# Bergvca/string_grouper

Hardware: NVIDIA H100
Metric: match_strings matched pairs/sec (663k names self-match @0.8, top 20, 3-gram) (higher is better)
Workload: dtype f64

## Files before the change

### string_grouper_b200/csrc/sg_cossim.cu

```cuda
#include <cub/cub.cuh>
#include <cuda_fp16.h>

#include "sg_common.cuh"

namespace sg {

constexpr int PB_THREADS = 1024;
constexpr int PB_ITEMS = 8;
constexpr int PB_CAP = PB_THREADS * PB_ITEMS;
constexpr size_t PB_SMEM = (size_t)PB_CAP * 8;

__device__ __forceinline__ uint32_t make_posting(float v, float w_scale, uint32_t local) {
    return ((uint32_t)__half_as_ushort(__float2half_rn(v * w_scale)) << 16) | local;
}

__global__ void postings_tile_count_kernel(int64_t n_rows, int64_t T, int W, const int64_t *__restrict__ indptr,
                                           const int32_t *__restrict__ perm, int32_t *__restrict__ tile_cnt) {
    const int64_t t = (int64_t)blockIdx.x * (blockDim.x >> 5) + (threadIdx.x >> 5);
    if (t > T) return;
    int s = 0;
    if (t < T) {
        const int64_t p1 = (t + 1) * W < n_rows ? (t + 1) * W : n_rows;
        for (int64_t p = t * W + lane_id(); p < p1; p += 32) {
            const int64_t row = perm ? perm[p] : p;
            s += (int)(indptr[row + 1] - indptr[row]);
        }
    }
#pragma unroll
    for (int o = 16; o; o >>= 1) s += __shfl_xor_sync(FULL, s, o);
    if (lane_id() == 0) tile_cnt[t] = s;
}

__device__ __forceinline__ void postings_emit_runs(const uint32_t *keys, const uint32_t *pst, int n, int start,
                                                   int64_t t, int64_t T, int64_t Tp, int2 *__restrict__ dir,
                                                   unsigned short *__restrict__ maxw_rows) {
    for (int i = threadIdx.x; i < n; i += blockDim.x) {
        const uint32_t f = keys[i];
        if (i > 0 && keys[i - 1] == f) continue;
        uint32_t m = 0;
        int j = i;
        for (; j < n && keys[j] == f; ++j) m = max(m, (pst[j] >> 16) & 0x7fffu);
        dir[(int64_t)f * T + t] = make_int2(start + i, (int)(((uint32_t)(j - i) & 0xffffu) | (m << 16)));
        maxw_rows[(int64_t)f * Tp + t] = (unsigned short)m;
    }
}

template <int ITEMS>
__device__ __forceinline__ void postings_sort_tile(uint32_t *skey, uint32_t *spost, int n, int key_bits) {
    typedef cub::BlockRadixSort<uint32_t, PB_THREADS, ITEMS, uint32_t> Sort;
    static_assert(sizeof(typename Sort::TempStorage) <= PB_SMEM, "block sort scratch exceeds the tile buffers");
    const uint32_t pad = (uint32_t)((1ull << key_bits) - 1);
    uint32_t keys[ITEMS], vals[ITEMS];
#pragma unroll
    for (int k = 0; k < ITEMS; ++k) {
        const int i = k * PB_THREADS + threadIdx.x;
        keys[k] = i < n ? skey[i] : pad;
        vals[k] = i < n ? spost[i] : 0u;
    }
    __syncthreads();
    Sort(*reinterpret_cast<typename Sort::TempStorage *>(skey)).SortBlockedToStriped(keys, vals, 0, key_bits);
    __syncthreads();
#pragma unroll
    for (int k = 0; k < ITEMS; ++k) {
        const int i = k * PB_THREADS + threadIdx.x;
        skey[i] = keys[k];
        spost[i] = vals[k];
    }
}

__global__ void __launch_bounds__(PB_THREADS)
postings_tile_build_kernel(int64_t n_rows, int64_t T, int64_t Tp, int W, int key_bits,
                           const int64_t *__restrict__ indptr, const int32_t *__restrict__ indices,
                           const float *__restrict__ val, const int32_t *__restrict__ perm, float w_scale,
                           const int32_t *__restrict__ tile_off, uint32_t *__restrict__ post, int2 *__restrict__ dir,
                           unsigned short *__restrict__ maxw_rows, uint32_t *__restrict__ big_key,
                           uint32_t *__restrict__ big_post, int32_t *__restrict__ big_end, int32_t *n_spilled) {
    typedef cub::BlockScan<int, PB_THREADS> Scan;
    __shared__ typename Scan::TempStorage scan_tmp;
    __shared__ int64_t row_p0[PB_THREADS];
    __shared__ int row_off[PB_THREADS];
    extern __shared__ __align__(16) uint32_t pb_smem[];
    uint32_t *skey = pb_smem, *spost = pb_smem + PB_CAP;

    const int64_t t = blockIdx.x;
    const int off0 = tile_off[t], n = tile_off[t + 1] - off0;
    const bool big = n > PB_CAP;
    if (threadIdx.x == 0) {
        big_end[t] = big ? off0 + n : off0;
        if (big && n_spilled) atomicAdd(n_spilled, 1);
    }
    uint32_t *kdst = big ? big_key + off0 : skey, *pdst = big ? big_post + off0 : spost;

    const int64_t p0 = t * W;
    const int nr = (int)((p0 + W < n_rows ? p0 + W : n_rows) - p0);
    int base = 0;
    for (int r0 = 0; r0 < nr; r0 += PB_THREADS) {
        const int r = r0 + threadIdx.x;
        int len = 0;
        int64_t q = 0;
        if (r < nr) {
            const int64_t row = perm ? perm[p0 + r] : p0 + r;
            q = indptr[row];
            len = (int)(indptr[row + 1] - q);
        }
        int o, total;
        Scan(scan_tmp).ExclusiveSum(len, o, total);
        row_p0[threadIdx.x] = q;
        row_off[threadIdx.x] = o;
        __syncthreads();
#pragma unroll 4
        for (int j = threadIdx.x; j < total; j += PB_THREADS) {
            int k = 0;
#pragma unroll
            for (int s = PB_THREADS / 2; s; s >>= 1)
                if (row_off[k + s] <= j) k += s;
            const int64_t p = row_p0[k] + (j - row_off[k]);
            kdst[base + j] = (uint32_t)indices[p];
            pdst[base + j] = make_posting(val[p], w_scale, (uint32_t)(r0 + k));
        }
        base += total;
        __syncthreads();
    }
    if (big) return;

    if (n <= PB_THREADS * 2) postings_sort_tile<2>(skey, spost, n, key_bits);
    else if (n <= PB_THREADS * 4) postings_sort_tile<4>(skey, spost, n, key_bits);
    else postings_sort_tile<PB_ITEMS>(skey, spost, n, key_bits);
    __syncthreads();
    for (int i = threadIdx.x; i < n; i += PB_THREADS) post[off0 + i] = spost[i];
    postings_emit_runs(skey, spost, n, off0, t, T, Tp, dir, maxw_rows);
}

__global__ void __launch_bounds__(256)
postings_big_dir_kernel(int64_t T, int64_t Tp, const int32_t *__restrict__ tile_off,
                        const int32_t *__restrict__ big_end, const uint32_t *keys, const uint32_t *pst, uint32_t *post,
                        int2 *__restrict__ dir, unsigned short *__restrict__ maxw_rows) {
    const int64_t t = blockIdx.x;
    const int off0 = tile_off[t], n = big_end[t] - off0;
    if (n == 0) return;
    if (pst != post)
        for (int i = threadIdx.x; i < n; i += blockDim.x) post[off0 + i] = pst[off0 + i];
    postings_emit_runs(keys + off0, pst + off0, n, off0, t, T, Tp, dir, maxw_rows);
}

__device__ __forceinline__ float post_w(uint32_t e) { return __half2float(__ushort_as_half((unsigned short)(e >> 16))); }
__device__ __forceinline__ int post_c(uint32_t e) { return (int)(e & 0xffffu); }

__device__ __forceinline__ int dir_len(int2 d) { return d.y & 0xffff; }
__device__ __forceinline__ float dir_maxw(int2 d) {
    return __half2float(__ushort_as_half((unsigned short)((unsigned)d.y >> 16)));
}

constexpr int LONG_BUCKET = 64;
#ifndef SG_WALK_MLP
#define SG_WALK_MLP 1
#endif
#ifndef SG_FILTER_MLP
#define SG_FILTER_MLP 1
#endif

constexpr int min_ctas(int nw) { return nw == 32 ? 2 : nw == 16 ? 3 : nw == 8 ? 5 : 8; }

constexpr float FIX_ONE = 32768.f;

template <typename AccT>
struct AccOps;
template <>
struct AccOps<float> {
    typedef float val_t;
    static constexpr int PER16 = 4;
    static __device__ __forceinline__ float left_weight(float a) { return a; }
    static __device__ __forceinline__ float threshold(float thr) { return thr; }
    static __device__ __forceinline__ float fma_store(float *acc, int col, float a, float w) {
        const float v = fmaf(a, w, acc[col]);
        acc[col] = v;
        return v;
    }
    static __device__ __forceinline__ float atomic_add(float *acc, int col, float a, float w) {
        const float x = a * w;
        return atomicAdd(acc + col, x) + x;
    }
    static __device__ __forceinline__ float vmax(float a, float b) { return fmaxf(a, b); }
    static __device__ __forceinline__ unsigned above(const uint4 &v, float thr) {
        return (__uint_as_float(v.x) > thr ? 1u : 0u) | (__uint_as_float(v.y) > thr ? 2u : 0u) |
               (__uint_as_float(v.z) > thr ? 4u : 0u) | (__uint_as_float(v.w) > thr ? 8u : 0u);
    }
    static __device__ __forceinline__ float value(const uint4 &v, int i) {
        return __uint_as_float(i < 2 ? (i == 0 ? v.x : v.y) : (i == 2 ? v.z : v.w));
    }
};
template <>
struct AccOps<uint16_t> {
    typedef int val_t;
    static constexpr int PER16 = 8;
    static __device__ __forceinline__ float left_weight(float a) { return a * FIX_ONE; }
    static __device__ __forceinline__ int threshold(float thr) { return (int)floorf(thr * FIX_ONE); }
    static __device__ __forceinline__ int atomic_add(uint16_t *acc, int col, float a, float w) {
        const int x = __float2int_rn(a * w);
        const unsigned sh = ((unsigned)col & 1u) << 4;
        const unsigned old = atomicAdd(reinterpret_cast<unsigned *>(acc) + (col >> 1), (unsigned)x << sh);
        return (int)((old >> sh) & 0xffffu) + x;
    }
    static __device__ __forceinline__ int fma_store(uint16_t *acc, int col, float a, float w) {
        return atomic_add(acc, col, a, w);
    }
    static __device__ __forceinline__ int vmax(int a, int b) { return max(a, b); }
    static __device__ __forceinline__ unsigned pair_above(unsigned u, int thr) {
        return ((int)(u & 0xffffu) > thr ? 1u : 0u) | ((int)(u >> 16) > thr ? 2u : 0u);
    }
    static __device__ __forceinline__ unsigned above(const uint4 &v, int thr) {
        return pair_above(v.x, thr) | (pair_above(v.y, thr) << 2) | (pair_above(v.z, thr) << 4) |
               (pair_above(v.w, thr) << 6);
    }
    static __device__ __forceinline__ float value(const uint4 &v, int i) {
        const unsigned w = i < 4 ? (i < 2 ? v.x : v.y) : (i < 6 ? v.z : v.w);
        return (float)((w >> ((i & 1) << 4)) & 0xffffu) * (1.f / FIX_ONE);
    }
};

template <typename AccT>
__device__ __forceinline__ void apply_buckets(AccT *__restrict__ acc, const uint32_t *__restrict__ post, int b0,
                                              int len, float a, int lane,
                                              typename AccOps<AccT>::val_t &seen) {
    typedef AccOps<AccT> Ops;
    unsigned m = __ballot_sync(FULL, len >= LONG_BUCKET);
    while (m) {
        const int src = __ffs(m) - 1;
        m &= m - 1;
        const int s = __shfl_sync(FULL, b0, src);
        const int e = s + __shfl_sync(FULL, len, src);
        const float ak = __shfl_sync(FULL, a, src);
        int p = s + lane;
        for (; p + 96 < e; p += 128) {
            const uint32_t e0 = post[p], e1 = post[p + 32], e2 = post[p + 64], e3 = post[p + 96];
            const typename Ops::val_t v0 = Ops::fma_store(acc, post_c(e0), ak, post_w(e0));
            const typename Ops::val_t v1 = Ops::fma_store(acc, post_c(e1), ak, post_w(e1));
            const typename Ops::val_t v2 = Ops::fma_store(acc, post_c(e2), ak, post_w(e2));
            const typename Ops::val_t v3 = Ops::fma_store(acc, post_c(e3), ak, post_w(e3));
            seen = Ops::vmax(Ops::vmax(Ops::vmax(seen, v0), Ops::vmax(v1, v2)), v3);
        }
        for (; p < e; p += 32) {
            const uint32_t e0 = post[p];
            seen = Ops::vmax(seen, Ops::fma_store(acc, post_c(e0), ak, post_w(e0)));
        }
        __syncwarp();
    }
    const int ln = len >= LONG_BUCKET ? 0 : len;
    int incl = ln;
#pragma unroll
    for (int o = 1; o < 32; o <<= 1) {
        const int up = __shfl_up_sync(FULL, incl, o);
        if (lane >= o) incl += up;
    }
    const int total = __shfl_sync(FULL, incl, 31);
    const int d = b0 - (incl - ln);
    for (int base = 0; base < total; base += 32 * SG_WALK_MLP) {
        uint32_t e[SG_WALK_MLP];
        float ak[SG_WALK_MLP];
#pragma unroll
        for (int u = 0; u < SG_WALK_MLP; ++u) {
            const int item = base + 32 * u + lane;
            int k = 0;
#pragma unroll
            for (int st = 16; st; st >>= 1) {
                const int v = __shfl_sync(FULL, incl, k + st - 1);
                if (v <= item) k += st;
            }
            const int dk = __shfl_sync(FULL, d, k);
            ak[u] = __shfl_sync(FULL, a, k);
            e[u] = 0u;
            if (item < total) e[u] = post[dk + item];
        }
#pragma unroll
        for (int u = 0; u < SG_WALK_MLP; ++u) {
            const int item = base + 32 * u + lane;
            if (item < total) seen = Ops::vmax(seen, Ops::atomic_add(acc, post_c(e[u]), ak[u], post_w(e[u])));
        }
    }
    __syncwarp();
}

struct FloorArgs {
    float *floor;
    const int32_t *self_rank;
    int seed, top_n;
    float margin, margin_pf;
};

__device__ __forceinline__ void floor_merge(float &kept, float x, int lane) {
#pragma unroll
    for (int k = 2; k <= 32; k <<= 1) {
#pragma unroll
        for (int j = k >> 1; j > 0; j >>= 1) {
            const float o = __shfl_xor_sync(FULL, x, j);
            x = (((lane & k) == 0) == ((lane & j) == 0)) ? fminf(x, o) : fmaxf(x, o);
        }
    }
    kept = fmaxf(kept, x);
#pragma unroll
    for (int j = 16; j > 0; j >>= 1) {
        const float o = __shfl_xor_sync(FULL, kept, j);
        kept = (lane & j) == 0 ? fmaxf(kept, o) : fminf(kept, o);
    }
}

template <int NW, typename AccT, bool FLOOR, bool RANGE = false>
__device__ __forceinline__ void
candidates_body(const int64_t *__restrict__ a_indptr, const int32_t *__restrict__ a_len,
                const int32_t *__restrict__ a_idx, const float *__restrict__ a_val, int64_t row_begin,
                int64_t row_end, const int32_t *__restrict__ perm_a, int64_t n_right,
                const int2 *__restrict__ bdir, const uint32_t *__restrict__ maxw_h,
                const uint32_t *__restrict__ post, const int32_t *__restrict__ perm_b, int Tp, int W,
                int64_t T, int64_t tiles_per_group, float a_scale, float thr_all,
                const float *__restrict__ thr_row, const float *__restrict__ xp_norm,
                const float *__restrict__ tile_bound, const int32_t *__restrict__ diag_rank,
                const unsigned long long *__restrict__ group_items, int32_t *__restrict__ cand_row,
                int32_t *__restrict__ cand_col, float *__restrict__ cand_partial, unsigned long long cap,
                unsigned long long *__restrict__ cand_count, unsigned long long *__restrict__ row_queue,
                const FloorArgs &fa, const int32_t *__restrict__ hi_pos = nullptr) {
    typedef AccOps<AccT> Ops;
    typedef typename Ops::val_t val_t;
    extern __shared__ __align__(16) unsigned char smem_raw[];
    const int lane = threadIdx.x & 31;
    const int warp = threadIdx.x >> 5;
    AccT *acc = reinterpret_cast<AccT *>(smem_raw) + (size_t)warp * W;
    uint4 *acc16 = reinterpret_cast<uint4 *>(acc);
    const int n16 = W / Ops::PER16;
    const uint4 zero4 = make_uint4(0u, 0u, 0u, 0u);

    for (int c = lane; c < n16; c += 32) acc16[c] = zero4;
    __syncwarp();

    const int64_t n_rows = row_end - row_begin;
    const int64_t n_groups = (T + tiles_per_group - 1) / tiles_per_group;
    unsigned long long n_items =
        group_items ? group_items[n_groups] : (unsigned long long)n_rows * (unsigned long long)n_groups;
    if constexpr (FLOOR) {
        if (fa.self_rank) n_items = (unsigned long long)n_rows * (unsigned long long)(fa.seed ? 1 : n_groups - 1);
    }
    const int n_tiles = (int)T;
    int64_t group = 0;
    for (;;) {
        unsigned long long item = 0;
        if (lane == 0) item = atomicAdd(row_queue, 1ull);
        item = __shfl_sync(FULL, item, 0);
        if (item >= n_items) break;
        int64_t ridx;
        if (group_items) {
            while (item >= group_items[group + 1]) ++group;
            ridx = (int64_t)(item - group_items[group]);
            if constexpr (RANGE) ridx += (int64_t)group_items[n_groups + 1 + group];
        } else {
            group = (int64_t)(item / (unsigned long long)n_rows);
            ridx = (int64_t)(item % (unsigned long long)n_rows);
        }
        const int64_t row = perm_a ? perm_a[ridx] : row_begin + ridx;
        int own_batch = 0;
        if constexpr (FLOOR) {
            if (fa.self_rank) {
                const int64_t pos = fa.self_rank[row];
                const int64_t own = pos / (tiles_per_group * W);
                if (fa.seed) {
                    group = own;
                    own_batch = (int)((pos / W - own * tiles_per_group) >> 6);
                } else if (group >= own) {
                    ++group;
                }
            }
        }
        const int64_t p0 = a_indptr[row];
        const int nf = a_len ? a_len[row] : (int)(a_indptr[row + 1] - p0);
        if (nf == 0) continue;
        float thr_r = thr_row ? thr_row[row] : thr_all;
        float e_r = 0.f, kept = 0.f, floor_seen = 0.f;
        if constexpr (FLOOR) e_r = __fmaf_ru(fa.margin_pf, (float)nf, fa.margin);
        const float xp = xp_norm ? xp_norm[row] : 0.f;
        const int t_begin = (int)(group * tiles_per_group);
        int t_end = (int)(t_begin + tiles_per_group < T ? t_begin + tiles_per_group : T);
        const int dr = diag_rank ? diag_rank[row] : 0;
        int hr = 0;
        if constexpr (RANGE) {
            hr = hi_pos[row];
            const int t_hi = (int)(((int64_t)hr + W - 1) / W);
            if (t_hi < t_end) t_end = t_hi;
        }
        const int t_first = (int)(((int64_t)dr / W) & ~63);
        const int tb_begin = t_first > t_begin ? t_first : t_begin;

        int f0 = 0;
        float a0 = 0.f;
        __half2 a2 = __float2half2_rn(0.f);
        if (lane < nf) {
            f0 = a_idx[p0 + lane];
            const float a = a_val[p0 + lane] * a_scale;
            a0 = Ops::left_weight(a);
            a2 = __half2half2(__float2half_ru(fabsf(a)));
        }
        const int2 *drow = bdir + f0 * n_tiles;
        const int nk = nf < 32 ? nf : 32;
        const float slack = 5e-4f * (float)nf + 1e-4f;

        for (int tb0 = tb_begin; tb0 < t_end; tb0 += 64) {
            int tb = tb0;
            if constexpr (FLOOR) {
                tb += own_batch * 64;
                if (tb >= t_end) tb -= (t_end - tb_begin + 63) / 64 * 64;
                const float f = __shfl_sync(FULL, __ldcg(fa.floor + row), 0);
                if (f > floor_seen) {
                    floor_seen = f;
                    thr_r = fmaxf(thr_r, __fsub_rd(__fsub_rd(f, e_r), FLOOR_EPS));
                }
            }
            unsigned m_even, m_odd;
            const int t0 = tb + 2 * lane;
            const bool up0 = (t0 + 1) * W > dr, up1 = (t0 + 2) * W > dr;
            {
                __half2 ub2 = __float2half2_rn(0.f);
                const uint32_t *mrow = maxw_h + (tb >> 1) + lane;
                for (int k0 = 0; k0 < nk; k0 += SG_FILTER_MLP) {
                    uint32_t m[SG_FILTER_MLP];
                    __half2 ak2[SG_FILTER_MLP];
#pragma unroll
                    for (int u = 0; u < SG_FILTER_MLP; ++u) {
                        const int kk = k0 + u;
                        const int fk = __shfl_sync(FULL, f0, kk & 31);
                        ak2[u] = __shfl_sync(FULL, a2, kk & 31);
                        m[u] = kk < nk ? mrow[fk * (Tp >> 1)] : 0u;
                    }
#pragma unroll
                    for (int u = 0; u < SG_FILTER_MLP; ++u)
                        ub2 = __hfma2(ak2[u], *reinterpret_cast<const __half2 *>(&m[u]), ub2);
                }
                for (int base = 32; base < nf; base += 32) {
                    int fl = 0;
                    __half2 al = __float2half2_rn(0.f);
                    if (base + lane < nf) {
                        fl = a_idx[p0 + base + lane];
                        al = __half2half2(__float2half_ru(fabsf(a_val[p0 + base + lane] * a_scale)));
                    }
                    const int nc = nf - base < 32 ? nf - base : 32;
                    for (int kk = 0; kk < nc; ++kk) {
                        const int fk = __shfl_sync(FULL, fl, kk);
                        const __half2 ak = __shfl_sync(FULL, al, kk);
                        const uint32_t mv = mrow[fk * (Tp >> 1)];
                        ub2 = __hfma2(ak, *reinterpret_cast<const __half2 *>(&mv), ub2);
                    }
                }
                const float2 ub = __half22float2(ub2);
                const float2 tb2 = reinterpret_cast<const float2 *>(tile_bound)[(tb >> 1) + lane];
                const float thr0 = xp > 0.f ? fmaxf(fmaf(-xp, tb2.x, thr_r), 0.f) : thr_r;
                const float thr1 = xp > 0.f ? fmaxf(fmaf(-xp, tb2.y, thr_r), 0.f) : thr_r;
                m_even = __ballot_sync(FULL, t0 < t_end && up0 && ub.x + slack > thr0);
                m_odd = __ballot_sync(FULL, t0 + 1 < t_end && up1 && ub.y + slack > thr1);
            }
            int t = -1;
            if (m_even) { t = tb + 2 * (__ffs(m_even) - 1); m_even &= m_even - 1; }
            else if (m_odd) { t = tb + 2 * (__ffs(m_odd) - 1) + 1; m_odd &= m_odd - 1; }
            int2 d_cur = make_int2(0, 0);
            if (t >= 0 && lane < nf) d_cur = drow[t];
            while (t >= 0) {
                int t_next = -1;
                if (m_even) { t_next = tb + 2 * (__ffs(m_even) - 1); m_even &= m_even - 1; }
                else if (m_odd) { t_next = tb + 2 * (__ffs(m_odd) - 1) + 1; m_odd &= m_odd - 1; }
                int2 d_next = make_int2(0, 0);
                if (t_next >= 0 && lane < nf) d_next = drow[t_next];

                const float thr_f = xp > 0.f ? fmaxf(fmaf(-xp, tile_bound[t], thr_r), 0.f) : thr_r;
                const val_t thr_c = Ops::threshold(thr_f);
                val_t seen = 0;
                apply_buckets<AccT>(acc, post, d_cur.x, dir_len(d_cur), a0, lane, seen);
                if (nf > 32) {
                    for (int base = 32; base < nf; base += 32) {
                        const int k = base + lane;
                        int b0 = 0, len = 0;
                        float a = 0.f;
                        if (k < nf) {
                            const int2 d = bdir[a_idx[p0 + k] * n_tiles + t];
                            a = Ops::left_weight(a_val[p0 + k] * a_scale);
                            b0 = d.x;
                            len = dir_len(d);
                        }
                        apply_buckets<AccT>(acc, post, b0, len, a, lane, seen);
                    }
                }
                if (!__any_sync(FULL, seen > thr_c)) {
                    for (int c = lane; c < n16; c += 32) acc16[c] = zero4;
                } else {
                    for (int c0 = 0; c0 < n16; c0 += 32) {
                        const int c = c0 + lane;
                        unsigned m = 0;
                        uint4 v = zero4;
                        if (c < n16) {
                            v = acc16[c];
                            if (v.x | v.y | v.z | v.w) {
                                acc16[c] = zero4;
                                m = Ops::above(v, thr_c);
                                const int below = dr - (t * W + c * Ops::PER16);
                                if (below > 0) m = below >= Ops::PER16 ? 0u : m & (~0u << below);
                                if constexpr (RANGE) {
                                    const int room = hr - (t * W + c * Ops::PER16);
                                    if (room < Ops::PER16) m = room <= 0 ? 0u : m & ((1u << room) - 1u);
                                }
                            }
                        }
                        if constexpr (FLOOR) {
                            float best = 0.f;
                            for (unsigned mm = m; mm; mm &= mm - 1) best = fmaxf(best, Ops::value(v, __ffs(mm) - 1));
                            const float lb = fmaxf(__fsub_rd(best, e_r), 0.f);
                            if (__any_sync(FULL, lb > __shfl_sync(FULL, kept, fa.top_n - 1))) {
                                floor_merge(kept, lb, lane);
                                const float kth = __shfl_sync(FULL, kept, fa.top_n - 1);
                                if (kth > floor_seen) {
                                    floor_seen = kth;
                                    if (lane == 0) atomicMax(reinterpret_cast<int *>(fa.floor + row), __float_as_int(kth));
                                    thr_r = fmaxf(thr_r, __fsub_rd(__fsub_rd(kth, e_r), FLOOR_EPS));
                                }
                            }
                        }
                        if (__any_sync(FULL, m != 0)) {
                            const int cnt = __popc(m);
                            int incl = cnt;
#pragma unroll
                            for (int o = 1; o < 32; o <<= 1) {
                                const int up = __shfl_up_sync(FULL, incl, o);
                                if (lane >= o) incl += up;
                            }
                            unsigned long long slot = 0;
                            if (lane == 31) slot = atomicAdd(cand_count, (unsigned long long)incl);
                            slot = __shfl_sync(FULL, slot, 31) + (unsigned long long)(incl - cnt);
                            while (m) {
                                const int i = __ffs(m) - 1;
                                m &= m - 1;
                                if (slot < cap) {
                                    const int col = t * W + c * Ops::PER16 + i;
                                    cand_row[slot] = (int32_t)row;
                                    cand_col[slot] = perm_b ? perm_b[col] : col;
                                    if (cand_partial) cand_partial[slot] = Ops::value(v, i);
                                }
                                ++slot;
                            }
                        }
                    }
                }
                __syncwarp();
                t = t_next;
                d_cur = d_next;
            }
        }
    }
}

#define SG_CAND_PARAMS                                                                                              \
    const int64_t *__restrict__ a_indptr, const int32_t *__restrict__ a_len, const int32_t *__restrict__ a_idx,     \
        const float *__restrict__ a_val, int64_t row_begin, int64_t row_end, const int32_t *__restrict__ perm_a,    \
        int64_t n_right, const int2 *__restrict__ bdir, const uint32_t *__restrict__ maxw_h,                        \
        const uint32_t *__restrict__ post, const int32_t *__restrict__ perm_b, int Tp, int W, int64_t T,            \
        int64_t tiles_per_group, float a_scale, float thr_all, const float *__restrict__ thr_row,                   \
        const float *__restrict__ xp_norm, const float *__restrict__ tile_bound,                                    \
        const int32_t *__restrict__ diag_rank, const unsigned long long *__restrict__ group_items,                  \
        int32_t *__restrict__ cand_row, int32_t *__restrict__ cand_col, float *__restrict__ cand_partial,           \
        unsigned long long cap, unsigned long long *__restrict__ cand_count,                                        \
        unsigned long long *__restrict__ row_queue
#define SG_CAND_ARGS                                                                                              \
    a_indptr, a_len, a_idx, a_val, row_begin, row_end, perm_a, n_right, bdir, maxw_h, post, perm_b, Tp, W, T,     \
        tiles_per_group, a_scale, thr_all, thr_row, xp_norm, tile_bound, diag_rank, group_items, cand_row,        \
        cand_col, cand_partial, cap, cand_count, row_queue

template <int NW, typename AccT>
__global__ void __launch_bounds__(NW * 32, min_ctas(NW)) cossim_candidates_kernel(SG_CAND_PARAMS) {
    candidates_body<NW, AccT, false>(SG_CAND_ARGS, FloorArgs{});
}

template <int NW, typename AccT>
__global__ void __launch_bounds__(NW * 32, min_ctas(NW)) cossim_candidates_floor_kernel(SG_CAND_PARAMS, FloorArgs fa) {
    candidates_body<NW, AccT, true>(SG_CAND_ARGS, fa);
}

template <int NW, typename AccT>
__global__ void __launch_bounds__(NW * 32, min_ctas(NW))
    cossim_candidates_range_kernel(SG_CAND_PARAMS, const int32_t *__restrict__ hi_pos) {
    candidates_body<NW, AccT, false, true>(SG_CAND_ARGS, FloorArgs{}, hi_pos);
}
#undef SG_CAND_PARAMS
#undef SG_CAND_ARGS

__global__ void diag_last_kernel(int64_t n_rows, const int32_t *__restrict__ perm_a, int64_t row_begin,
                                 const int32_t *__restrict__ diag_rank, int64_t group_cols,
                                 unsigned long long *__restrict__ last) {
    const int64_t ridx = (int64_t)blockIdx.x * blockDim.x + threadIdx.x;
    long long g = -1;
    if (ridx < n_rows) g = diag_rank[perm_a ? perm_a[ridx] : row_begin + ridx] / group_cols;
    const unsigned peers = __match_any_sync(FULL, g);
    if (g >= 0 && lane_id() == 31 - __clz(peers)) atomicMax(last + g, (unsigned long long)(ridx + 1));
}

__global__ void diag_items_kernel(int64_t n_groups, unsigned long long *__restrict__ items) {
    const int lane = threadIdx.x;
    unsigned long long run_max = 0, run_sum = 0;
    for (int64_t g0 = 0; g0 < n_groups; g0 += 32) {
        const int64_t g = g0 + lane;
        unsigned long long v = g < n_groups ? items[g] : 0ull;
#pragma unroll
        for (int o = 1; o < 32; o <<= 1) {
            const unsigned long long up = __shfl_up_sync(FULL, v, o);
            if (lane >= o && up > v) v = up;
        }
        if (run_max > v) v = run_max;
        run_max = __shfl_sync(FULL, v, 31);
        if (g >= n_groups) v = 0;
        unsigned long long s = v;
#pragma unroll
        for (int o = 1; o < 32; o <<= 1) {
            const unsigned long long up = __shfl_up_sync(FULL, s, o);
            if (lane >= o) s += up;
        }
        if (g < n_groups) items[g] = run_sum + s - v;
        run_sum += __shfl_sync(FULL, s, 31);
    }
    if (lane == 0) items[n_groups] = run_sum;
}

__global__ void range_groups_kernel(int64_t n_rows, const int32_t *__restrict__ perm_a, int64_t row_begin,
                                    const int32_t *__restrict__ lo_pos, const int32_t *__restrict__ hi_pos,
                                    int64_t group_cols, int64_t n_groups, unsigned long long *__restrict__ items) {
    const int64_t ridx = (int64_t)blockIdx.x * blockDim.x + threadIdx.x;
    long long g0 = -1, g1 = -1;
    if (ridx < n_rows) {
        const int64_t row = perm_a ? perm_a[ridx] : row_begin + ridx;
        const int64_t lo = lo_pos[row], hi = hi_pos[row];
        if (hi > lo) {
            g0 = lo / group_cols;
            g1 = (hi - 1) / group_cols;
        }
    }
    unsigned peers = __match_any_sync(FULL, g0);
    if (g0 >= 0 && lane_id() == 31 - __clz(peers)) atomicMax(items + g0, (unsigned long long)(ridx + 1));
    peers = __match_any_sync(FULL, g1);
    if (g1 >= 0 && lane_id() == __ffs(peers) - 1)
        atomicMax(items + n_groups + 1 + g1, (unsigned long long)(n_rows - ridx));
}

__global__ void range_items_kernel(int64_t n_rows, int64_t n_groups, unsigned long long *__restrict__ items) {
    const int lane = threadIdx.x;
    unsigned long long *first = items + n_groups + 1;
    unsigned long long run = 0;
    for (int64_t g0 = 0; g0 < n_groups; g0 += 32) {
        const int64_t g = n_groups - 1 - g0 - lane;
        unsigned long long v = g >= 0 ? first[g] : 0ull;
#pragma unroll
        for (int o = 1; o < 32; o <<= 1) {
            const unsigned long long up = __shfl_up_sync(FULL, v, o);
            if (lane >= o && up > v) v = up;
        }
        if (run > v) v = run;
        run = __shfl_sync(FULL, v, 31);
        if (g >= 0) first[g] = (unsigned long long)n_rows - v;
    }
    unsigned long long run_max = 0, run_sum = 0;
    for (int64_t g0 = 0; g0 < n_groups; g0 += 32) {
        const int64_t g = g0 + lane;
        unsigned long long v = g < n_groups ? items[g] : 0ull;
#pragma unroll
        for (int o = 1; o < 32; o <<= 1) {
            const unsigned long long up = __shfl_up_sync(FULL, v, o);
            if (lane >= o && up > v) v = up;
        }
        if (run_max > v) v = run_max;
        run_max = __shfl_sync(FULL, v, 31);
        const unsigned long long c = (g < n_groups && v > first[g]) ? v - first[g] : 0ull;
        unsigned long long s = c;
#pragma unroll
        for (int o = 1; o < 32; o <<= 1) {
            const unsigned long long up = __shfl_up_sync(FULL, s, o);
            if (lane >= o) s += up;
        }
        if (g < n_groups) items[g] = run_sum + s - c;
        run_sum += __shfl_sync(FULL, s, 31);
    }
    if (lane == 0) items[n_groups] = run_sum;
}

template <typename T>
struct ExactOps;
template <>
struct ExactOps<double> {
    static __device__ __forceinline__ double mul(double a, double b) { return __dmul_rn(a, b); }
    static __device__ __forceinline__ double add(double a, double b) { return __dadd_rn(a, b); }
};
template <>
struct ExactOps<float> {
    static __device__ __forceinline__ float mul(float a, float b) { return __fmul_rn(a, b); }
    static __device__ __forceinline__ float add(float a, float b) { return __fadd_rn(a, b); }
};

template <typename T>
__device__ __forceinline__ T merge_dot(const int32_t *__restrict__ ai, const T *__restrict__ av, int64_t pa,
                                       int64_t ea, const int32_t *__restrict__ bi,
                                       const T *__restrict__ bv, int64_t pb, int64_t eb) {
    T sum = (T)0;
    if (pa >= ea || pb >= eb) return sum;
    int32_t fa = ai[pa], fb = bi[pb];
    for (;;) {
        if (fa == fb) {
            sum = ExactOps<T>::add(sum, ExactOps<T>::mul(av[pa], bv[pb]));
            ++pa;
            ++pb;
            if (pa >= ea || pb >= eb) break;
            fa = ai[pa];
            fb = bi[pb];
        } else if (fa < fb) {
            if (++pa >= ea) break;
            fa = ai[pa];
        } else {
            if (++pb >= eb) break;
            fb = bi[pb];
        }
    }
    return sum;
}

template <typename T>
__device__ __forceinline__ T merge_dot_vec(const int32_t *__restrict__ ai, const T *__restrict__ av, int64_t pa,
                                           int64_t ea, const int32_t *__restrict__ bi,
                                           const T *__restrict__ bv, int64_t pb, int64_t eb) {
    T sum = (T)0;
    if (pa >= ea || pb >= eb) return sum;
    const int32_t END = 0x7fffffff;
    int32_t fa = ai[pa];
    for (int64_t k = pb & ~(int64_t)3; k < eb; k += 4) {
        int32_t f[4];
        if (k + 4 <= eb) {
            const int4 q = __ldg(reinterpret_cast<const int4 *>(bi + k));
            f[0] = q.x, f[1] = q.y, f[2] = q.z, f[3] = q.w;
        } else {
#pragma unroll
            for (int j = 0; j < 4; ++j) f[j] = k + j < eb ? bi[k + j] : END;
        }
#pragma unroll
        for (int j = 0; j < 4; ++j) {
            const int64_t p = k + j;
            if (p < pb || p >= eb) continue;
            const int32_t fb = f[j];
            while (fa < fb) {
                if (++pa >= ea) return sum;
                fa = ai[pa];
            }
            if (fa == fb) sum = ExactOps<T>::add(sum, ExactOps<T>::mul(av[pa], bv[p]));
        }
    }
    return sum;
}

__device__ __forceinline__ void keep_pairs(bool keep, bool mir, int32_t r, int32_t c, double sc, int lane,
                                           int32_t *__restrict__ keep_row, int32_t *__restrict__ keep_col,
                                           double *__restrict__ out, unsigned long long *__restrict__ keep_count,
                                           unsigned long long *__restrict__ mirror_count,
                                           int32_t *__restrict__ row_cnt, int64_t row_begin) {
    const unsigned m = __ballot_sync(FULL, keep);
    if (!m) return;
    const unsigned mm = __ballot_sync(FULL, mir);
    const int leader = __ffs(m) - 1;
    unsigned long long base = 0;
    if (lane == leader) {
        base = atomicAdd(keep_count, (unsigned long long)(__popc(m) + __popc(mm)));
        if (mm) atomicAdd(mirror_count, (unsigned long long)__popc(mm));
    }
// ... 891 lines not shown
```

Measured before the change: 218.1 million.

## Widen block-max filter to four tiles per lane in non-floor path

Generalizes the tile upper-bound filter so each lane evaluates TPL tiles (4 when FLOOR is off, 2 when on), loading maxw entries as uint2 and doing two half2 FMAs per feature. This halves the number of filter iterations and shuffles per tile when FLOOR is off, and widens the per-lane loads. It also adds an SG_BLOCKMAX_ONLY compile-time probe that counts passing tiles. The risks are more registers and a changed order of candidate tiles. The FLOOR path still steps own_batch by 64 while BATCH is 64 there, so that path is unchanged in size.

```diff
diff --git a/string_grouper_b200/csrc/sg_cossim.cu b/string_grouper_b200/csrc/sg_cossim.cu
--- a/string_grouper_b200/csrc/sg_cossim.cu
+++ b/string_grouper_b200/csrc/sg_cossim.cu
@@ -1,5 +1,7 @@
 #include <cub/cub.cuh>
 #include <cuda_fp16.h>
+
+#include <type_traits>
 
 #include "sg_common.cuh"
 
@@ -304,6 +306,29 @@
     }
 }
 
+template <int TPL>
+__device__ __forceinline__ void bound_fma(__half2 (&ub2)[TPL / 2], __half2 a, uint32_t m) {
+    ub2[0] = __hfma2(a, *reinterpret_cast<const __half2 *>(&m), ub2[0]);
+}
+template <int TPL>
+__device__ __forceinline__ void bound_fma(__half2 (&ub2)[TPL / 2], __half2 a, uint2 m) {
+    ub2[0] = __hfma2(a, *reinterpret_cast<const __half2 *>(&m.x), ub2[0]);
+    ub2[1] = __hfma2(a, *reinterpret_cast<const __half2 *>(&m.y), ub2[1]);
+}
+
+template <int TPL>
+__device__ __forceinline__ int next_tile(unsigned (&mk)[TPL], int tb) {
+    int t = -1;
+#pragma unroll
+    for (int c = 0; c < TPL; ++c) {
+        if (t < 0 && mk[c]) {
+            t = tb + TPL * (__ffs(mk[c]) - 1) + c;
+            mk[c] &= mk[c] - 1;
+        }
+    }
+    return t;
+}
+
 template <int NW, typename AccT, bool FLOOR, bool RANGE = false>
 __device__ __forceinline__ void
 candidates_body(const int64_t *__restrict__ a_indptr, const int32_t *__restrict__ a_len,
@@ -320,6 +345,8 @@
                 const FloorArgs &fa, const int32_t *__restrict__ hi_pos = nullptr) {
     typedef AccOps<AccT> Ops;
     typedef typename Ops::val_t val_t;
+    constexpr int TPL = FLOOR ? 2 : 4;
+    constexpr int BATCH = 32 * TPL;
     extern __shared__ __align__(16) unsigned char smem_raw[];
     const int lane = threadIdx.x & 31;
     const int warp = threadIdx.x >> 5;
@@ -339,12 +366,20 @@
         if (fa.self_rank) n_items = (unsigned long long)n_rows * (unsigned long long)(fa.seed ? 1 : n_groups - 1);
     }
     const int n_tiles = (int)T;
+#ifdef SG_BLOCKMAX_ONLY
+    unsigned long long n_pass = 0;
+#endif
     int64_t group = 0;
     for (;;) {
         unsigned long long item = 0;
         if (lane == 0) item = atomicAdd(row_queue, 1ull);
         item = __shfl_sync(FULL, item, 0);
-        if (item >= n_items) break;
+        if (item >= n_items) {
+#ifdef SG_BLOCKMAX_ONLY
+            if (lane == 0) atomicAdd(cand_count, n_pass);
+#endif
+            break;
+        }
         int64_t ridx;
         if (group_items) {
             while (item >= group_items[group + 1]) ++group;
@@ -400,7 +435,7 @@
         const int nk = nf < 32 ? nf : 32;
         const float slack = 5e-4f * (float)nf + 1e-4f;
 
-        for (int tb0 = tb_begin; tb0 < t_end; tb0 += 64) {
+        for (int tb0 = tb_begin; tb0 < t_end; tb0 += BATCH) {
             int tb = tb0;
             if constexpr (FLOOR) {
                 tb += own_batch * 64;
@@ -411,25 +446,27 @@
                     thr_r = fmaxf(thr_r, __fsub_rd(__fsub_rd(f, e_r), FLOOR_EPS));
                 }
             }
-            unsigned m_even, m_odd;
-            const int t0 = tb + 2 * lane;
-            const bool up0 = (t0 + 1) * W > dr, up1 = (t0 + 2) * W > dr;
+            unsigned mk[TPL];
+            const int t0 = tb + TPL * lane;
             {
-                __half2 ub2 = __float2half2_rn(0.f);
-                const uint32_t *mrow = maxw_h + (tb >> 1) + lane;
+                typedef typename std::conditional<TPL == 4, uint2, uint32_t>::type mword;
+                __half2 ub2[TPL / 2];
+#pragma unroll
+                for (int c = 0; c < TPL / 2; ++c) ub2[c] = __float2half2_rn(0.f);
+                const mword *mrow = reinterpret_cast<const mword *>(maxw_h) + tb / TPL + lane;
+                const int fstride = Tp / TPL;
                 for (int k0 = 0; k0 < nk; k0 += SG_FILTER_MLP) {
-                    uint32_t m[SG_FILTER_MLP];
+                    mword m[SG_FILTER_MLP];
                     __half2 ak2[SG_FILTER_MLP];
 #pragma unroll
                     for (int u = 0; u < SG_FILTER_MLP; ++u) {
                         const int kk = k0 + u;
                         const int fk = __shfl_sync(FULL, f0, kk & 31);
                         ak2[u] = __shfl_sync(FULL, a2, kk & 31);
-                        m[u] = kk < nk ? mrow[fk * (Tp >> 1)] : 0u;
+                        m[u] = kk < nk ? mrow[fk * fstride] : mword{};
                     }
 #pragma unroll
-                    for (int u = 0; u < SG_FILTER_MLP; ++u)
-                        ub2 = __hfma2(ak2[u], *reinterpret_cast<const __half2 *>(&m[u]), ub2);
+                    for (int u = 0; u < SG_FILTER_MLP; ++u) bound_fma<TPL>(ub2, ak2[u], m[u]);
                 }
                 for (int base = 32; base < nf; base += 32) {
                     int fl = 0;
@@ -442,26 +479,27 @@
                     for (int kk = 0; kk < nc; ++kk) {
                         const int fk = __shfl_sync(FULL, fl, kk);
                         const __half2 ak = __shfl_sync(FULL, al, kk);
-                        const uint32_t mv = mrow[fk * (Tp >> 1)];
-                        ub2 = __hfma2(ak, *reinterpret_cast<const __half2 *>(&mv), ub2);
+                        bound_fma<TPL>(ub2, ak, mrow[fk * fstride]);
                     }
                 }
-                const float2 ub = __half22float2(ub2);
-                const float2 tb2 = reinterpret_cast<const float2 *>(tile_bound)[(tb >> 1) + lane];
-                const float thr0 = xp > 0.f ? fmaxf(fmaf(-xp, tb2.x, thr_r), 0.f) : thr_r;
-                const float thr1 = xp > 0.f ? fmaxf(fmaf(-xp, tb2.y, thr_r), 0.f) : thr_r;
-                m_even = __ballot_sync(FULL, t0 < t_end && up0 && ub.x + slack > thr0);
-                m_odd = __ballot_sync(FULL, t0 + 1 < t_end && up1 && ub.y + slack > thr1);
+#pragma unroll
+                for (int c = 0; c < TPL; ++c) {
+                    const float ub = c & 1 ? __high2float(ub2[c >> 1]) : __low2float(ub2[c >> 1]);
+                    const float bd = t0 + c < t_end ? tile_bound[t0 + c] : 0.f;
+                    const float thr = xp > 0.f ? fmaxf(fmaf(-xp, bd, thr_r), 0.f) : thr_r;
+                    mk[c] = __ballot_sync(FULL, t0 + c < t_end && (t0 + c + 1) * W > dr && ub + slack > thr);
+                }
             }
-            int t = -1;
-            if (m_even) { t = tb + 2 * (__ffs(m_even) - 1); m_even &= m_even - 1; }
-            else if (m_odd) { t = tb + 2 * (__ffs(m_odd) - 1) + 1; m_odd &= m_odd - 1; }
+#ifdef SG_BLOCKMAX_ONLY
+#pragma unroll
+            for (int c = 0; c < TPL; ++c) n_pass += __popc(mk[c]);
+            continue;
+#endif
+            int t = next_tile<TPL>(mk, tb);
             int2 d_cur = make_int2(0, 0);
             if (t >= 0 && lane < nf) d_cur = drow[t];
             while (t >= 0) {
-                int t_next = -1;
-                if (m_even) { t_next = tb + 2 * (__ffs(m_even) - 1); m_even &= m_even - 1; }
-                else if (m_odd) { t_next = tb + 2 * (__ffs(m_odd) - 1) + 1; m_odd &= m_odd - 1; }
+                const int t_next = next_tile<TPL>(mk, tb);
                 int2 d_next = make_int2(0, 0);
                 if (t_next >= 0 && lane < nf) d_next = drow[t_next];
 
```

After: 247.8 million, median of 6. +13.6%, better.
